# steineggerlab/Metabuli

Hardware: AMD Instinct MI355X
Metric: Mreads/s classified (metabuli classify hot path, reads + index resident in HBM) (higher is better)
Workload: dtype u64

## Files before the change

metabuli_amd/csrc/kernels_score_fast.h:

```cpp
#ifndef MTB_KERNELS_SCORE_FAST_H
#define MTB_KERNELS_SCORE_FAST_H
#include "dev_util.h"
#include "kernels_score.h"
#include "mtb_core.h"
#include "mtb_score_par.h"

#define MTB_FAST_BKT 128
#ifndef MTB_FAST_MERGE_SINGLES
#define MTB_FAST_MERGE_SINGLES 0
#endif

#ifdef MTB_FAST_DEBUG
__device__ unsigned long long mtb_fast_reasons[32];
#define MTB_FAST_COUNT(k, v) do { if (threadIdx.x == 0) atomicAdd(&mtb_fast_reasons[k], (unsigned long long)(v)); } while (0)
#define MTB_FAST_T0() unsigned long long ft_ = __builtin_readcyclecounter()
#define MTB_FAST_MARK(k) do { const unsigned long long t_ = __builtin_readcyclecounter(); if (threadIdx.x == 0) s_ph[k] += t_ - ft_; ft_ = t_; } while (0)
#else
#define MTB_FAST_COUNT(k, v) do {} while (0)
#define MTB_FAST_T0() do {} while (0)
#define MTB_FAST_MARK(k) do {} while (0)
#endif

#define MTB_DPP_RED(v, OP) do { \
    { const uint32_t o_ = (uint32_t)__builtin_amdgcn_update_dpp((int)(v), (int)(v), 0x111, 0xF, 0xF, false); (v) = OP((v), o_); } \
    { const uint32_t o_ = (uint32_t)__builtin_amdgcn_update_dpp((int)(v), (int)(v), 0x112, 0xF, 0xF, false); (v) = OP((v), o_); } \
    { const uint32_t o_ = (uint32_t)__builtin_amdgcn_update_dpp((int)(v), (int)(v), 0x114, 0xF, 0xF, false); (v) = OP((v), o_); } \
    { const uint32_t o_ = (uint32_t)__builtin_amdgcn_update_dpp((int)(v), (int)(v), 0x118, 0xF, 0xF, false); (v) = OP((v), o_); } \
    { const uint32_t o_ = (uint32_t)__builtin_amdgcn_update_dpp((int)(v), (int)(v), 0x142, 0xA, 0xF, false); (v) = OP((v), o_); } \
    { const uint32_t o_ = (uint32_t)__builtin_amdgcn_update_dpp((int)(v), (int)(v), 0x143, 0xC, 0xF, false); (v) = OP((v), o_); } } while (0)
#define MTB_MINU(a, b) ((b) < (a) ? (b) : (a))
#define MTB_MAXU(a, b) ((b) > (a) ? (b) : (a))
__device__ __forceinline__ uint32_t wave_min_u32(uint32_t v) { MTB_DPP_RED(v, MTB_MINU); return (uint32_t)__builtin_amdgcn_readlane((int)v, 63); }
__device__ __forceinline__ uint32_t wave_max_u32(uint32_t v) { MTB_DPP_RED(v, MTB_MAXU); return (uint32_t)__builtin_amdgcn_readlane((int)v, 63); }

struct FKey { uint32_t lo, hi; };
__device__ __forceinline__ uint32_t fk_species(const FKey &k) { return k.hi >> 10; }
__device__ __forceinline__ uint32_t fk_frame(const FKey &k) { return (k.hi >> 7) & 7u; }
__device__ __forceinline__ uint32_t fk_pos(const FKey &k) { return ((k.hi & 127u) << 4) | (k.lo >> 27); }
__device__ __forceinline__ uint32_t fk_ham(const FKey &k) { return (k.lo >> 24) & 7u; }
__device__ __forceinline__ uint32_t fk_dna(const FKey &k) { return k.lo & 0xFFFFFFu; }

struct FastPath { int32_t start, end; float score; int32_t ham; uint32_t rehs;  int32_t species; };

template <int K, int KL = K, bool BYFRAME = false>
__global__ __launch_bounds__(64, K <= 3 ? 5 : 4) void k_score_fast(const mtb_slot16 *__restrict__ slots_all, uint64_t n_reads, const int32_t *__restrict__ qlen,
                                                       const int32_t *__restrict__ qlen2, mtb_tax_view tx, mtb_score_params sp,
                                                       const uint64_t *__restrict__ tc_off, mtb_result *__restrict__ results,
                                                       int32_t *__restrict__ tc_tax, uint32_t *__restrict__ tc_cnt, uint64_t tc_cap, uint64_t tc_base,
                                                       const uint32_t *__restrict__ cursor, uint32_t stride, uint32_t direct, uint32_t epoch,
                                                       uint8_t *__restrict__ slow_flag, uint32_t *__restrict__ cnt_out) {
    constexpr int NMAX = 64 * K;
    __shared__ FKey s_key[NMAX];
    __shared__ uint64_t s_aux[NMAX];
    __shared__ uint64_t s_pp[NMAX];
    __shared__ FastPath s_path[64];
    __shared__ uint32_t s_pf[64];
    __shared__ uint32_t s_tl[(BYFRAME || MTB_FAST_MERGE_SINGLES) ? 64 : 1];
    typedef uint32_t __attribute__((may_alias)) u32a; typedef int32_t __attribute__((may_alias)) i32a;
    static_assert(NMAX * 8 >= 2 * MTB_FAST_BKT * 4 && NMAX * 8 >= 256 * 4 && NMAX * 8 >= (MTB_LR_MAXE + MTB_LR_MAXE * MTB_LR_K) * 4, "tables fit the arrays they live in");
    u32a *const s_hcnt = (u32a *)s_pp;
    u32a *const s_hmin = (u32a *)s_key; i32a *const s_btax = (i32a *)s_key + MTB_FAST_BKT;
    i32a *const s_otax = (i32a *)s_pp; u32a *const s_ocnt = (u32a *)s_pp + MTB_FAST_BKT;
    i32a *const s_lev = (i32a *)s_aux; i32a *const s_anc = (i32a *)s_aux + MTB_LR_MAXE;
    const int32_t lane = (int32_t)threadIdx.x;
    MTB_BEGIN_ACQUIRE();
#ifdef MTB_FAST_DEBUG
    __shared__ unsigned long long s_ph[16];
    if (threadIdx.x < 16) s_ph[threadIdx.x] = 0;
#endif
    const uint64_t lt = lanemask_lt();
    const uint64_t le = lt | (1ull << lane);
    const uint32_t tail_cap = stride - direct;
    const uint32_t div_m = (65536u + (uint32_t)sp.dna_shift - 1u) / (uint32_t)sp.dna_shift;
    const uint32_t lines = (stride * (uint32_t)sizeof(mtb_slot16) + 127u) / 128u;

    for (uint64_t r = blockIdx.x; r < n_reads; r += gridDim.x) {
        if (r + gridDim.x < n_reads && (uint32_t)lane < lines) {
            const uint8_t *pf = (const uint8_t *)(slots_all + (r + gridDim.x) * (uint64_t)stride) + (uint64_t)lane * 128u;
            __builtin_amdgcn_global_load_lds((const __attribute__((address_space(1))) void *)pf, (__attribute__((address_space(3))) void *)s_pf, 4, 0, 0);
        }
        MTB_FAST_T0();
        const int32_t ql1 = qlen[r], ql2 = qlen2[r];
        const int32_t read_len = ql1 + ql2;
        const int32_t nb = mtb_num_buckets(read_len, sp.dna_shift);
        const uint32_t cur = cursor[r];
        const mtb_slot16 *slots = slots_all + r * (uint64_t)stride;
        mtb_slot16 x[KL];
#pragma unroll
        for (int k = 0; k < KL; k++) { const uint32_t i = (uint32_t)lane + 64u * k; x[k].a = 0; x[k].b = 0; if (i < stride) x[k] = slots[i]; }
        bool slow = cur > tail_cap || nb > MTB_FAST_BKT;
        wave_fence();
        MTB_FAST_MARK(0);
        int32_t n = 0, n_live = 0;
        uint32_t spc[KL]; bool live[KL]; int32_t dst[KL];
        uint32_t smin = 0xFFFFFFFFu, smax = 0u;
#pragma unroll
        for (int k = 0; k < KL; k++) {
            const uint32_t i = (uint32_t)lane + 64u * k;
            live[k] = i < stride && mtb_slot_epoch(x[k]) == epoch && (i < direct || i - direct < cur);
            spc[k] = live[k] ? (uint32_t)(x[k].a >> 32) : 0xFFFFFFFFu;
            dst[k] = 0;
            n_live += (int32_t)__popcll(__ballot(live[k]));
            smin = spc[k] < smin ? spc[k] : smin;
            if (live[k]) smax = spc[k] > smax ? spc[k] : smax;
        }
        smin = wave_min_u32(smin); smax = wave_max_u32(smax);
        uint32_t todo_min = 0xFFFFFFFFu;
        if (smin != smax) {
            for (int32_t q = lane; q < 256; q += 64) s_hcnt[q] = 0;
            wave_fence();
#pragma unroll
            for (int k = 0; k < KL; k++) if (live[k]) atomicAdd(&s_hcnt[(spc[k] * 0x9E3779B1u) >> 24], 1u);
            wave_fence();
#pragma unroll
            for (int k = 0; k < KL; k++) if (live[k] && s_hcnt[(spc[k] * 0x9E3779B1u) >> 24] < 2u) { live[k] = false; spc[k] = 0xFFFFFFFFu; }
        } else if (n_live < 2) {
#pragma unroll
            for (int k = 0; k < KL; k++) { live[k] = false; spc[k] = 0xFFFFFFFFu; }
        }
        if (BYFRAME) {
#pragma unroll
            for (int k = 0; k < KL; k++) if (live[k]) spc[k] = (spc[k] << 3) | ((uint32_t)(x[k].b >> 52) & 7u);
        }
#pragma unroll
        for (int k = 0; k < KL; k++) todo_min = spc[k] < todo_min ? spc[k] : todo_min;
        for (int round = 0; ; round++) {
            const uint32_t m = wave_min_u32(todo_min);
            if (m == 0xFFFFFFFFu) break;
            if (round == 24) { slow = true; break; }
            todo_min = 0xFFFFFFFFu;
#pragma unroll
            for (int k = 0; k < KL; k++) {
                const bool mine = spc[k] == m;
                const uint64_t mask = __ballot(mine);
                if (mine) { dst[k] = n + (int32_t)__popcll(mask & lt); spc[k] = 0xFFFFFFFFu; }
                n += (int32_t)__popcll(mask);
                todo_min = spc[k] < todo_min ? spc[k] : todo_min;
            }
        }
        if (KL > K && n > NMAX) slow = true;
#pragma unroll
        for (int k = 0; k < KL; k++) {
            if (live[k] && !slow) {
                const uint64_t b = x[k].b;
                const uint32_t bh = (uint32_t)(b >> 32), ps_ = (bh >> 8) & 0x7FFu;
                FKey fk; fk.hi = ((uint32_t)(x[k].a >> 32) << 10) | (((bh >> 20) & 7u) << 7) | (ps_ >> 4);
                fk.lo = ((ps_ & 15u) << 27) | (((bh >> 23) & 7u) << 24) | ((uint32_t)b & 0xFFFFFFu);
                s_key[dst[k]] = fk;
                s_aux[dst[k]] = (x[k].a & 0xFFFFFFFFull) | (((b >> 24) & 0xFFFFull) << 32) | ((uint32_t)lane + 64u * k >= direct ? (1ull << 63) : 0ull);
            }
        }
        MTB_FAST_MARK(1);
        mtb_result R = mtb_result_blank(ql1, ql2, (uint32_t)tc_base);
        if (!slow && n == 0) { if (lane == 0) { cnt_out[r] = (uint32_t)n_live; results[r] = R; } continue; }
        wave_fence();
        {
            uint32_t nt = 0;
            bool any_tail = false;
#pragma unroll
            for (int k = 0; k < KL; k++) any_tail |= live[k] && (uint32_t)lane + 64u * k >= direct;
            if ((BYFRAME || MTB_FAST_MERGE_SINGLES) && !slow && __any(any_tail)) {
                FKey ke[K]; uint64_t ax[K]; int32_t np[K]; bool tl[K];
                const int32_t nsl = (n + 63) >> 6;
#pragma unroll
                for (int k = 0; k < K; k++) {
                    const int32_t i = lane + 64 * k;
                    ke[k].lo = 0; ke[k].hi = 0; ax[k] = 0; np[k] = i; tl[k] = false;
                    if (k < nsl && i < n) { ke[k] = s_key[i]; ax[k] = s_aux[i]; tl[k] = (ax[k] >> 63) != 0; }
                    if (k < nsl) {
                        const uint64_t tm = __ballot(tl[k]);
                        if (tl[k]) { const uint32_t at = nt + (uint32_t)__popcll(tm & lt); if (at < 64u) s_tl[at] = (uint32_t)i; }
                        nt += (uint32_t)__popcll(tm);
                    }
                }
                if (nt > 64u) slow = true;
                wave_fence();
                if (!slow) {
                    auto same_run = [&](const FKey &a, const FKey &b) { return BYFRAME ? ((a.hi ^ b.hi) >> 7) == 0 : ((a.hi ^ b.hi) >> 10) == 0; };
                    auto less = [&](const FKey &a, const FKey &b) { return a.hi < b.hi || (a.hi == b.hi && a.lo < b.lo); };
                    for (uint32_t t = 0; t < nt; t++) {
                        const int32_t ti = (int32_t)s_tl[t];
                        const FKey kt = s_key[ti];
                        uint32_t n_dir_less = 0, n_dir_run = 0;
#pragma unroll
                        for (int k = 0; k < K; k++) {
                            if (k < nsl) {
                                const int32_t i = lane + 64 * k;
                                const bool dir = i < n && !tl[k] && same_run(ke[k], kt);
                                const bool smaller = dir && less(ke[k], kt);
                                if (dir && !smaller) np[k]++;
                                n_dir_run += (uint32_t)__popcll(__ballot(dir)); n_dir_less += (uint32_t)__popcll(__ballot(smaller));
                            }
                        }
                        uint32_t n_tl_less = 0, n_tl_before = 0;
                        for (uint32_t u = 0; u < nt; u++) {
                            if (u == t) continue;
                            const FKey ku = s_key[s_tl[u]];
                            if (!same_run(ku, kt)) continue;
                            n_tl_less += (less(ku, kt) || (!less(kt, ku) && u < t)) ? 1u : 0u; n_tl_before += u < t ? 1u : 0u;
                        }
                        const int32_t run_start = ti - (int32_t)n_dir_run - (int32_t)n_tl_before;
#pragma unroll
                        for (int k = 0; k < K; k++) if (lane + 64 * k == ti) np[k] = run_start + (int32_t)(n_dir_less + n_tl_less);
                    }
                    wave_fence();
#pragma unroll
                    for (int k = 0; k < K; k++) { const int32_t i = lane + 64 * k; if (k < nsl && i < n) { s_key[np[k]] = ke[k]; s_aux[np[k]] = ax[k] & ~(1ull << 63); } }
                    wave_fence();
                }
            }
        }
        FKey key[K]; uint32_t tid[K], reh[K];
        int32_t tcanon[K]; uint8_t euk[K];
        const mtb_tax_node *nodes = (const mtb_tax_node *)tx.node;
        bool bhead[K], linked[K];
        int32_t shv[K];
        uint64_t bmask[K + 1], lmask[K + 1], rmask[K];
        const int32_t nslot = (n + 63) >> 6;
        bool bad = false, bad2 = false;
#ifdef MTB_FAST_DEBUG
        if (slow) MTB_FAST_COUNT(cur > tail_cap || nb > MTB_FAST_BKT ? 0 : 1, 1);
#endif
#pragma unroll
        for (int k = 0; k < K; k++) {
            const int32_t i = lane + 64 * k;
            key[k].lo = 0; key[k].hi = 0; tid[k] = 0; reh[k] = 0; bhead[k] = true; linked[k] = false; shv[k] = 0; tcanon[k] = -1; euk[k] = 0;
            bmask[k] = ~0ull; lmask[k] = 0; rmask[k] = 0;
            if (k < nslot && !slow) {
                FKey pk; pk.lo = 0; pk.hi = 0;
                if (i < n) {
                    key[k] = s_key[i]; const uint64_t a = s_aux[i]; tid[k] = (uint32_t)a; reh[k] = (uint32_t)(a >> 32) & 0xFFFFu; if (i > 0) pk = s_key[i - 1];
                }
                {
                    const int32_t t_ = (int32_t)tid[k], s_ = (int32_t)fk_species(key[k]);
                    const bool tv = i < n && t_ >= 0 && t_ <= tx.max_taxid, sv = i < n && s_ >= 0 && s_ <= tx.max_taxid;
                    const int32_t tc_ = nodes[tv ? t_ : 0].canon; const uint8_t eu_ = tx.under_euk[sv ? s_ : 0];
                    tcanon[k] = tv ? tc_ : -1; euk[k] = sv ? eu_ : 0;
                }
                const bool first = i == 0;
                if (i < n && !first) {
                    if (pk.hi > key[k].hi || (pk.hi == key[k].hi && pk.lo > key[k].lo)) bad = true;
                    if (pk.hi == key[k].hi && ((pk.lo ^ key[k].lo) >> 27) == 0) bad2 = true;
                }
                bhead[k] = i >= n || first || ((pk.hi ^ key[k].hi) >> 7) != 0;
                if (i < n && !bhead[k]) {
                    const int32_t pos = (int32_t)fk_pos(key[k]), ppos = (int32_t)fk_pos(pk);
                    const int32_t s = (pos - ppos) / 3;
                    if (s > 0 && s <= sp.max_codon_shift) {
                        shv[k] = s;
                        const bool fwd = fk_frame(key[k]) < 3u;
                        linked[k] = mtb_consecutive(fk_dna(pk), fk_dna(key[k]), s, fwd, sp.kmer_format);
                    }
                }
                bmask[k] = __ballot(bhead[k]);
                lmask[k] = __ballot(linked[k]);
                rmask[k] = __ballot(i < n && !linked[k]);
            }
        }
        bmask[K] = ~0ull; lmask[K] = 0;
#ifdef MTB_FAST_DEBUG
        if (!slow) { if (__any(bad)) MTB_FAST_COUNT(2, 1); else if (__any(bad2)) MTB_FAST_COUNT(3, 1); }
#endif
        slow = slow || __any(bad || bad2);
        if (slow) { if (lane == 0) slow_flag[r] = cur > tail_cap ? 2 : 1; continue; }
        if (lane == 0) cnt_out[r] = (uint32_t)n_live;
        MTB_FAST_MARK(2);
        float ps[K]; int32_t phd[K]; int32_t root[K];
        bool cand[K];
        {
            float carry_s = 0.0f; int32_t carry_hd = 0, last_root = 0;
#pragma unroll
            for (int k = 0; k < K; k++) {
                ps[k] = 0.0f; phd[k] = 0; root[k] = 0; cand[k] = false;
                if (k < nslot) {
                    const int32_t i = lane + 64 * k;
                    float is = 0.0f; int32_t ihd = 0;
                    if (linked[k]) mtb_link_inc(reh[k], shv[k], &is, &ihd);
                    ps[k] = wave_inclusive_scan_dpp(is) + carry_s; phd[k] = wave_inclusive_scan_dpp(ihd) + carry_hd;
                    carry_s = rl_f(ps[k], 63); carry_hd = rl_i(phd[k], 63);
                    const uint64_t mr = rmask[k];
                    const uint64_t lo_roots = mr & le;
                    root[k] = lo_roots ? 64 * k + 63 - (int32_t)__builtin_clzll(lo_roots) : last_root;
                    if (mr) last_root = 64 * k + 63 - (int32_t)__builtin_clzll(mr);
                    if (i < n) s_pp[i] = (uint64_t)__float_as_uint(ps[k]) | ((uint64_t)(uint32_t)phd[k] << 32);
                    const uint64_t bnext = (bmask[k] >> 1) | ((bmask[k + 1] & 1ull) << 63);
                    const uint64_t lnext = (lmask[k] >> 1) | ((lmask[k + 1] & 1ull) << 63);
                    const bool has_next = !((bnext >> lane) & 1ull);
                    const bool conn = (lnext >> lane) & 1ull;
                    cand[k] = i < n && (!bhead[k] || has_next) && !conn;
                }
            }
        }
        wave_fence();
        MTB_FAST_MARK(3);
        int32_t ne = 0;
        bool too_many = false;
#pragma unroll
        for (int k = 0; k < K; k++) {
            if (k < nslot) {
                bool e = false;
                FastPath P; P.start = 0; P.end = 0; P.score = 0.0f; P.ham = 0; P.rehs = 0; P.species = 0;
                if (cand[k]) {
                    const int32_t spc = (int32_t)fk_species(key[k]);
                    const int32_t md = euk[k] ? sp.min_cons_cnt_euk : sp.min_cons_cnt;
                    const int32_t rt = root[k];
                    const uint64_t pr = s_pp[rt]; const FKey rkey = s_key[rt];
                    const uint32_t rreh = (uint32_t)(s_aux[rt] >> 32);
                    const int32_t dhd = phd[k] - (int32_t)(uint32_t)(pr >> 32);
                    const int32_t depth = 1 + mtb_link_depth(dhd);
                    if (depth >= md) {
                        e = true;
                        P.start = (int32_t)fk_pos(rkey);
                        P.end = (int32_t)fk_pos(key[k]) + 23;
                        P.score = mtb_part_score(rreh, 8, false) + (rt == lane + 64 * k ? 0.0f : ps[k] - __uint_as_float((uint32_t)pr));
                        P.ham = (int32_t)fk_ham(rkey) + (rt == lane + 64 * k ? 0 : mtb_link_ham(dhd));
                        P.rehs = rreh | (reh[k] << 16);
                        P.species = spc;
                    }
                }
                const uint64_t me = __ballot(e);
                const int32_t at = ne + (int32_t)__popcll(me & lt);
                if (e && at < 64) s_path[at] = P;
                ne += (int32_t)__popcll(me);
            }
        }
        too_many = ne > 64;
        if (too_many) MTB_FAST_COUNT(4, 1); else { MTB_FAST_COUNT(5, 1); MTB_FAST_COUNT(6, ne); }
        if (too_many) { if (lane == 0) slow_flag[r] = 1; continue; }
        if (ne == 0) { if (lane == 0) results[r] = R; continue; }
        wave_fence();
        MTB_FAST_MARK(4);
        FastPath P = s_path[lane < ne ? lane : 0];
        const bool have = lane < ne;
        int32_t prev_spc = __shfl_up(P.species, 1, 64);
        const bool shead = have && (lane == 0 || prev_spc != P.species);
        const uint64_t hmask = __ballot(shead);
        const int32_t nsp = (int32_t)__popcll(hmask);
        MTB_FAST_COUNT(7, nsp);

        float sp_score = -1.0f; int32_t sp_id = 0;
        int32_t s_idx = 0;
        const uint32_t ord = __float_as_uint(P.score);
        const uint32_t tie = ((uint32_t)(1023 - (P.ham < 1023 ? P.ham : 1023)) << 17) | ((uint32_t)(P.start & 0x7FF) << 6) | (uint32_t)(63 - lane);
        for (uint64_t hm = hmask; hm; hm &= hm - 1, s_idx++) {
            const int32_t slo = (int32_t)__builtin_ctzll(hm);
            const int32_t shi = (hm & (hm - 1)) ? (int32_t)__builtin_ctzll(hm & (hm - 1)) : ne;
            const bool in = lane >= slo && lane < shi;
            const uint32_t mh = wave_max_u32(in ? ord : 0u);
            const uint32_t ml = wave_max_u32(in && ord == mh ? tie : 0u);
            const int32_t bl = 63 - (int32_t)(ml & 63u);
            const int32_t f_st = rl_i(P.start, bl), f_en = rl_i(P.end, bl);
            bool surv = in;
            if (in && lane != bl && !((P.end < f_st) || (f_en < P.start))) {
                const int32_t ov = (P.end < f_en ? P.end : f_en) - (P.start > f_st ? P.start : f_st) + 1;
                if (mtb_overlap_drops(ov, P.end - P.start + 1)) surv = false;
            }
            const uint64_t smask = __ballot(surv);
            int32_t rank = 0;
            for (uint64_t fm = smask; fm; fm &= fm - 1) {
                const int32_t f = (int32_t)__builtin_ctzll(fm);
                const float fs = rl_f(P.score, f); const int32_t fh = rl_i(P.ham, f), fst = rl_i(P.start, f);
                const bool before = fs != P.score ? fs > P.score : (fh != P.ham ? fh < P.ham : (fst != P.start ? fst > P.start : f < lane));
                rank += (f != lane && before) ? 1 : 0;
            }
            const int32_t ns = (int32_t)__popcll(smask);
            int32_t acc_st = 0, acc_en = 0, na = 0; float sum = 0.0f;
            for (int32_t q = 0; q < ns; q++) {
                const int32_t o = (int32_t)__builtin_ctzll(__ballot(surv && rank == q));
                struct { int32_t start, end; float score; int32_t ham; } c;
                c.start = rl_i(P.start, o); c.end = rl_i(P.end, o); c.ham = rl_i(P.ham, o); c.score = rl_f(P.score, o);
                const uint32_t crehs = (uint32_t)rl_i((int32_t)P.rehs, o);
                bool drop = false;
                uint64_t ovm = __ballot(lane < na && !((c.end < acc_st) || (acc_en < c.start)));
                while (ovm && !drop) {
                    const int32_t a2 = (int32_t)__builtin_ctzll(ovm); ovm &= ovm - 1;
                    drop = mtb_path_against(c, rl_i(acc_st, a2), rl_i(acc_en, a2), [&] { return crehs >> 16; }, [&] { return crehs & 0xFFFFu; });
                }
                if (!drop) { if (lane == na) { acc_st = c.start; acc_en = c.end; } na++; sum += c.score; }
            }
            float sc = sum / (float)read_len; sc = sc < 1.0f ? sc : 1.0f;
            const int32_t spid = rl_i(P.species, slo);
            if (lane == s_idx) { sp_score = sc; sp_id = spid; }
        }
        MTB_FAST_MARK(5);
        const bool valid = lane < nsp && !(sp_score < sp.min_score);
        const int32_t meaningful = (int32_t)__popcll(__ballot(valid && sp_score > 0.0f));
        if (meaningful == 0) { if (lane == 0) results[r] = R; continue; }
        float best_sp = valid ? sp_score : -1.0f;
#pragma unroll
        for (int d = 32; d > 0; d >>= 1) { const float o2 = __shfl_xor(best_sp, d, 64); best_sp = o2 > best_sp ? o2 : best_sp; }
        const float cut = best_sp * sp.tie_ratio;
        mtb_tie tie_sp = mtb_tie_none();
        for (uint64_t tm = __ballot(valid && sp_score >= cut); tm; tm &= tm - 1) {
            const int32_t s = (int32_t)__builtin_ctzll(tm);
            mtb_tie_add(&tx, &tie_sp, rl_i(sp_id, s), rl_f(sp_score, s));
        }
        if (!mtb_tie_decide(&tie_sp, &sp, &R)) { if (lane == 0) results[r] = R; continue; }
        const int32_t species = tie_sp.only;
        const bool sp_ok = species >= 0 && species <= tx.max_taxid;
        mtb_tax_node rs = nodes[sp_ok ? species : 0];
        if (!sp_ok) { rs.canon = -1; rs.depth = 0; rs.parent = -1; rs.flags = 0; }
        MTB_FAST_MARK(6);
        for (int32_t q = lane; q < nb; q += 64) { s_hmin[q] = 255u; s_btax[q] = -1; }
        wave_fence();
        int32_t bq[K];
#pragma unroll
        for (int k = 0; k < K; k++) {
            bq[k] = -1;
            if (k < nslot) {
                const int32_t i = lane + 64 * k;
                if (i < n && (int32_t)fk_species(key[k]) == species) {
                    const int32_t q = (int32_t)((fk_pos(key[k]) * div_m) >> 16);
                    if (q < nb) { bq[k] = q; atomicMin(&s_hmin[q], fk_ham(key[k])); }
                }
            }
        }
        wave_fence();
#pragma unroll
        for (int k = 0; k < K; k++) {
            if (k < nslot && bq[k] >= 0 && fk_ham(key[k]) == s_hmin[bq[k]]) {
                const int32_t t = (int32_t)tid[k];
                const int32_t tc = tcanon[k] < 0 ? t : tcanon[k];
                mtb_bucket_merge(&s_btax[bq[k]], t, [&tx, tc](int32_t a, int32_t b) { return a == b ? tc : mtb_lca(&tx, a, b); });
            }
        }
        wave_fence();
        const uint64_t off = tc_off[r], room = tc_off[r + 1] - off;
        MTB_FAST_MARK(7);
        int32_t ntc = 0;
        {
            uint32_t t0 = 0xFFFFFFFFu, t1 = 0xFFFFFFFFu;
            if (lane < nb && s_hmin[lane] != 255u) t0 = (uint32_t)s_btax[lane];
            if (lane + 64 < nb && s_hmin[lane + 64] != 255u) t1 = (uint32_t)s_btax[lane + 64];
            while (ntc < (int32_t)room) {
                const uint32_t mn = wave_min_u32(t0 < t1 ? t0 : t1);
                if (mn == 0xFFFFFFFFu) break;
                const uint32_t cnt = (uint32_t)__popcll(__ballot(t0 == mn)) + (uint32_t)__popcll(__ballot(t1 == mn));
                if (lane == 0) { s_otax[ntc] = (int32_t)mn; s_ocnt[ntc] = cnt; }
                if (t0 == mn) t0 = 0xFFFFFFFFu;
                if (t1 == mn) t1 = 0xFFFFFFFFu;
                ntc++;
            }
        }
        wave_fence();
        MTB_FAST_MARK(8);
        int32_t slow_lr = ntc > MTB_LR_MAXE ? 1 : 0;
        if (!slow_lr && lane < ntc) {
            const int32_t tax = s_otax[lane];
            const bool t_ok = tax >= 0 && tax <= tx.max_taxid;
            mtb_tax_node rt = nodes[t_ok ? tax : 0];
            if (!t_ok) { rt.canon = -1; rt.depth = 0; rt.parent = -1; rt.flags = 0; }
            int32_t lv;
            const int32_t cs = rs.canon, c = rt.canon;
            if (cs < 0 || c < 0) lv = -1;
            else {
                const int32_t L = rt.depth - rs.depth;
                if (L < 0) lv = -1;
                else if (L > MTB_LR_K) lv = MTB_LR_K + 1;
                else {
                    int32_t a = c;
                    for (int32_t k = L - 1; k >= 0; k--) { s_anc[lane * MTB_LR_K + k] = a; a = (k == L - 1) ? rt.parent : tx.parent[a]; }
                    lv = (a == cs) ? L : -1;
                }
            }
            s_lev[lane] = lv;
            if (lv > MTB_LR_K) slow_lr = 1;
        }
        slow_lr = __any(slow_lr) ? 1 : 0;
        wave_fence();
        if (lane == 0) {
            R.n_taxcnt = (uint16_t)ntc;
            R.classification = mtb_finish_taxon(&tx, &sp, species, rs.canon, R.score, slow_lr != 0, s_lev, s_anc, s_otax, s_ocnt, ntc, read_len);
            R.taxcnt_off = (uint32_t)(off + tc_base);
            for (int32_t k = 0; k < ntc; k++)
                if (off + k < tc_cap) { tc_tax[off + k] = s_otax[k]; tc_cnt[off + k] = s_ocnt[k]; }
            results[r] = R;
        }
        MTB_FAST_MARK(9);
    }
#ifdef MTB_FAST_DEBUG
    __syncthreads();
    if (threadIdx.x < 16) atomicAdd(&mtb_fast_reasons[8 + threadIdx.x], s_ph[threadIdx.x]);
#endif
}

#endif
```

metabuli_amd/csrc/kernels_score_many.h:

```cpp
#ifndef MTB_KERNELS_SCORE_MANY_H
#define MTB_KERNELS_SCORE_MANY_H
#include "dev_util.h"
#include "mtb_core.h"
#include "kernels_join.h"
#include "kernels_score.h"
#include "kernels_score_long.h"
#include "kernels_seg_order.h"

#define MTB_MANY_CLAIM 16u
#define MTB_MANY_HASH 1024u

__global__ __launch_bounds__(256) void k_ovf_count(const uint32_t *__restrict__ cursor, const uint8_t *__restrict__ off, uint64_t n_reads, uint32_t tail_cap,
                                                    uint32_t *__restrict__ novf) {
    const uint64_t r = (uint64_t)blockIdx.x * 256 + threadIdx.x;
    if (r >= n_reads) return;
    const uint32_t cur = cursor[r];
    const uint32_t n = (cur > tail_cap && !(off && off[r])) ? cur - tail_cap : 0u;
    novf[r] = n <= 65535u ? n : 0u;
}
__global__ __launch_bounds__(256) void k_ovf_group(const mtb_match *__restrict__ ovf, uint64_t n_ovf, const uint64_t *__restrict__ start, const uint32_t *__restrict__ novf,
                                                    uint32_t *__restrict__ ocur, mtb_match *__restrict__ out, uint64_t region_cap, const unsigned long long *__restrict__ counters) {
    uint64_t i = (uint64_t)blockIdx.x * 256 + threadIdx.x;
    if (region_cap) {
        const unsigned long long cnt = counters[8 * blockIdx.y];
        if (i >= cnt || i >= region_cap) return;
        i += (uint64_t)blockIdx.y * region_cap;
    } else if (i >= n_ovf) return;
    mtb_match m = ovf[i];
    const uint32_t r = mtb_q_seq(m.qinfo) - 1;
    const uint32_t cap = novf[r];
    if (!cap) return;
    uint32_t at;
    if (m.pad & 2u) { at = (uint32_t)(m.qinfo >> 16) & 0xFFFFu; m.qinfo &= ~0xFFFF0000ull; m.pad = 0; }
    else at = atomicAdd(&ocur[r], 1u);
    if (at < cap) out[start[r] + at] = m;
}

#define MTB_MSORT_NT 256
template <int LOG2HASH, uint32_t MAXN>
__global__ __launch_bounds__(MTB_MSORT_NT) void k_many_sort(const mtb_slot16 *__restrict__ slots_all, uint32_t stride, uint32_t direct, uint32_t epoch,
                                                             const uint32_t *__restrict__ cursor, const uint8_t *__restrict__ off_reads,
                                                             const mtb_match *__restrict__ ovfg, const uint64_t *__restrict__ ovf_start,
                                                             const uint32_t *__restrict__ list, uint32_t n_list, const int32_t *__restrict__ qlen, const int32_t *__restrict__ qlen2,
                                                             int32_t dna_shift, const uint64_t *__restrict__ big_start, mtb_match *__restrict__ big, uint32_t *__restrict__ seg_cnt,
                                                             uint8_t *__restrict__ todo, uint32_t only_flag, uint32_t beyond_flag ) {
    constexpr uint32_t HASH = 1u << LOG2HASH;
    __shared__ __attribute__((aligned(16))) uint64_t s_u[HASH];
    __shared__ uint16_t s_idx[MAXN];
    __shared__ uint32_t s_n, s_full;
    static_assert(MAXN * 8 <= HASH * 8, "the sort keys live in the table's storage");
    uint32_t *const h_key = (uint32_t *)s_u, *const h_val = h_key + HASH;
    const uint32_t tid = threadIdx.x, lane = tid & 63u;
    const uint64_t lt = lanemask_lt();
    const uint32_t tail_cap = stride - direct;
    for (uint32_t b = blockIdx.x; b < n_list; b += gridDim.x) {
        const uint64_t r = (uint64_t)list[b];
        if (only_flag && todo[r] != only_flag) continue;
        const uint32_t cur = cursor[r], tail_n = cur < tail_cap ? cur : tail_cap;
        uint64_t o0 = 0; uint32_t n_ov = 0;
        if (ovf_start) { o0 = ovf_start[r]; n_ov = (uint32_t)(ovf_start[r + 1] - o0); }
        const int32_t nb = mtb_num_buckets(qlen[r] + qlen2[r], dna_shift);
        const bool skip = (off_reads && off_reads[r]) || cur - tail_n != n_ov || stride + n_ov > 65535u || nb > 256;
        __syncthreads();
        if (only_flag && tid == 0) todo[r] = 0;
        if (skip) { if (tid == 0) { seg_cnt[b] = 0; todo[r] = 1; } continue; }
        for (uint32_t q = tid; q < HASH; q += MTB_MSORT_NT) { h_key[q] = 0xFFFFFFFFu; h_val[q] = 0u; }
        if (tid == 0) { s_n = 0; s_full = 0; }
        __syncthreads();
        const mtb_slot16 *slots = slots_all + r * (uint64_t)stride;
        const uint32_t n_src = stride + n_ov;
        auto probe = [&](uint32_t i, uint32_t *sp_, uint32_t *fr_) -> bool {
            if (i < stride) { const mtb_slot16 x = slots[i]; *sp_ = (uint32_t)(x.a >> 32); *fr_ = (uint32_t)(x.b >> 52) & 7u; return seg_slot_live(x, i, direct, tail_n, epoch); }
            const mtb_match m = ovfg[o0 + (i - stride)]; *sp_ = (uint32_t)m.species_id; *fr_ = mtb_q_frame(m.qinfo); return true;
        };
        for (uint32_t i = tid; i < n_src; i += MTB_MSORT_NT) {
            uint32_t s_, f_;
            if (!probe(i, &s_, &f_)) continue;
            if (*(volatile uint32_t *)&s_full) break;
            uint32_t h = (s_ * 0x9E3779B1u) >> (32 - LOG2HASH); bool done = false;
            for (uint32_t p = 0; p < HASH && !done; p++) {
                const uint32_t old = atomicCAS(&h_key[h], 0xFFFFFFFFu, s_);
                if (old == 0xFFFFFFFFu || old == s_) { const uint32_t bit = 1u << f_; if (atomicOr(&h_val[h], bit) & bit) atomicOr(&h_val[h], bit << 8); done = true; }
                h = (h + 1u) & (HASH - 1u);
            }
            if (!done) s_full = 1;
        }
        __syncthreads();
        uint32_t used = 0;
        for (uint32_t q = tid; q < HASH; q += MTB_MSORT_NT) used += h_key[q] != 0xFFFFFFFFu ? 1u : 0u;
        if (used) atomicAdd(&s_n, used);
        __syncthreads();
        const bool over = s_full || s_n > HASH / 4u * 3u;
        __syncthreads();
        if (over) { if (tid == 0) { seg_cnt[b] = 0; todo[r] = (uint8_t)beyond_flag; } continue; }
        if (tid == 0) s_n = 0;
        __syncthreads();
        for (uint32_t i0 = 0; i0 < n_src; i0 += MTB_MSORT_NT) {
            const uint32_t i = i0 + tid;
            bool keep = false;
            if (i < n_src) {
                uint32_t s_, f_;
                if (probe(i, &s_, &f_)) {
                    uint32_t h = (s_ * 0x9E3779B1u) >> (32 - LOG2HASH);
                    for (uint32_t p = 0; p < HASH; p++) { const uint32_t k = h_key[h]; if (k == s_) { keep = (h_val[h] >> 8) != 0u; break; } if (k == 0xFFFFFFFFu) break; h = (h + 1u) & (HASH - 1u); }
                }
            }
            const uint64_t km = __ballot(keep);
            if (km) {
                uint32_t at0 = 0;
                if (lane == 0) at0 = atomicAdd(&s_n, (uint32_t)__popcll(km));
                at0 = (uint32_t)__shfl((int)at0, 0, 64);
                if (keep) { const uint32_t at = at0 + (uint32_t)__popcll(km & lt); if (at < MAXN) s_idx[at] = (uint16_t)i; }
            }
        }
        __syncthreads();
        const uint32_t n = s_n;
        __syncthreads();
        if (n > MAXN) { if (tid == 0) { seg_cnt[b] = 0; todo[r] = (uint8_t)beyond_flag; } continue; }
        auto fetch = [&](uint32_t i) -> mtb_match {
            if (i < stride) return mtb_slot_unpack(slots[i], (uint32_t)r + 1);
            mtb_match m = ovfg[o0 + (i - stride)]; m.pad = 0; return m;
        };
        for (uint32_t j = tid; j < n; j += MTB_MSORT_NT) {
            const mtb_match m = fetch(s_idx[j]);
            s_u[j] = ((uint64_t)(uint32_t)m.species_id << 41) | ((uint64_t)mtb_q_frame(m.qinfo) << 38) | ((uint64_t)(mtb_q_pos(m.qinfo) & 0x7FFu) << 27) |
                     ((uint64_t)(m.hamming & 7u) << 24) | (m.dna & 0xFFFFFFu);
        }
        __syncthreads();
        so_bitonic(s_u, s_idx, n, tid);
        mtb_match *dst = big + big_start[b];
        for (uint32_t j = tid; j < n; j += MTB_MSORT_NT) {
            const mtb_match m = fetch(s_idx[j]);
            uint64_t *d = (uint64_t *)(dst + j); const uint64_t *q = (const uint64_t *)&m;
            d[0] = q[0]; d[1] = q[1]; d[2] = q[2];
        }
        if (tid == 0) seg_cnt[b] = n;
    }
}
__global__ __launch_bounds__(256) void k_list_flagged(const uint32_t *__restrict__ list, uint32_t n_list, const uint8_t *__restrict__ todo, const uint32_t *__restrict__ big_cnt,
                                                       uint32_t *__restrict__ rest, uint32_t *__restrict__ n_rest, uint32_t *__restrict__ cnt_out) {
    const uint32_t b = blockIdx.x * 256 + threadIdx.x;
    if (b >= n_list) return;
    const uint32_t r = list[b];
    if (todo[r]) rest[atomicAdd(n_rest, 1u)] = r;
    else cnt_out[r] = big_cnt[b];
}

template <bool KEY64, int CAP>
__global__ __launch_bounds__(64, (CAP > 192 ? 2 : 3)) void k_score_many(const mtb_slot16 *__restrict__ slots_all, uint32_t stride, uint32_t direct, uint32_t epoch,
                                                       const uint32_t *__restrict__ cursor, const uint8_t *__restrict__ off_reads,
                                                       const mtb_match *__restrict__ ovfg, const uint64_t *__restrict__ ovf_start,
                                                       const uint32_t *__restrict__ list, const uint32_t *__restrict__ n_list,
                                                       const int32_t *__restrict__ qlen, const int32_t *__restrict__ qlen2, mtb_tax_view tx, mtb_score_params sp,
                                                       const uint64_t *__restrict__ tc_off, mtb_result *__restrict__ results, int32_t *__restrict__ tc_tax,
                                                       uint32_t *__restrict__ tc_cnt, uint64_t tc_cap, uint64_t tc_base,
                                                       uint32_t *__restrict__ rest_list, uint32_t *__restrict__ n_rest, uint32_t *__restrict__ cnt_out,
                                                       unsigned long long *__restrict__ work, unsigned long long *__restrict__ stats ) {
    __shared__ __attribute__((aligned(16))) uint8_t s_ws[MTB_SCORE_WS_BYTES_(CAP)];
    static_assert(MTB_SCORE_WS_BYTES_(CAP) - CAP * sizeof(mtb_match) >= MTB_MANY_HASH * 8, "the species table fits behind the match records");
    static_assert(CAP * sizeof(mtb_path) >= MTB_SCORE_BKT * 13 + (MTB_LR_MAXE + MTB_LR_MAXE * MTB_LR_K) * 4, "decide arrays must fit the path area");
    uint32_t *const h_key = (uint32_t *)(s_ws + CAP * sizeof(mtb_match));
    uint32_t *const h_val = h_key + MTB_MANY_HASH;
    __shared__ uint32_t s_tfull;
    const uint32_t lane = threadIdx.x;
    const uint64_t lt = lanemask_lt();
    const uint32_t tail_cap = stride - direct;
    MTB_BEGIN_ACQUIRE();
    const uint64_t n_iter = (uint64_t)*n_list;
    unsigned long long seen = 0, kept = 0;
    for (uint64_t c0 = (uint64_t)__shfl(lane == 0 ? atomicAdd(work, (unsigned long long)MTB_MANY_CLAIM) : 0ull, 0, 64); c0 < n_iter;
         c0 = (uint64_t)__shfl(lane == 0 ? atomicAdd(work, (unsigned long long)MTB_MANY_CLAIM) : 0ull, 0, 64))
    for (uint64_t it = c0; it < c0 + MTB_MANY_CLAIM && it < n_iter; it++) {
        const uint64_t r = (uint64_t)list[it];
        const int32_t ql1 = qlen[r], ql2 = qlen2[r];
        const int32_t read_len = ql1 + ql2;
        const int32_t nb = mtb_num_buckets(read_len, sp.dna_shift);
        const uint32_t cur = cursor[r];
        const uint32_t tail_n = cur < tail_cap ? cur : tail_cap;
        uint64_t o0 = 0; uint32_t n_ov = 0;
        if (ovf_start) { o0 = ovf_start[r]; n_ov = (uint32_t)(ovf_start[r + 1] - o0); }
        bool hand_on = (off_reads && off_reads[r]) || nb > MTB_SCORE_BKT || cur - tail_n != n_ov;
        uint32_t why = 2;
        if (!hand_on && cur > 3u * (uint32_t)CAP) { hand_on = true; why = 4; }
        const mtb_slot16 *slots = slots_all + r * (uint64_t)stride;
        mtb_sws<uint16_t> w;
        mtb_sws_carve<uint16_t>(&w, s_ws, CAP);
        uint32_t n = 0, n_all = 0;
        if (!hand_on) {
            score_sync<uint16_t>();
            for (uint32_t q = lane; q < MTB_MANY_HASH; q += 64) { h_key[q] = 0xFFFFFFFFu; h_val[q] = 0u; }
            if (lane == 0) s_tfull = 0;
            score_sync<uint16_t>();
            bool full = false;
            auto enter = [&](uint32_t s, uint32_t f) {
                if (*(volatile uint32_t *)&s_tfull) { full = true; return; }
                uint32_t h = (s * 0x9E3779B1u) >> 22;
                for (uint32_t p = 0; p < MTB_MANY_HASH; p++) {
                    const uint32_t old = atomicCAS(&h_key[h], 0xFFFFFFFFu, s);
                    if (old == 0xFFFFFFFFu || old == s) {
                        const uint32_t bit = 1u << f;
                        if (atomicOr(&h_val[h], bit) & bit) atomicOr(&h_val[h], bit << 8);
                        return;
                    }
                    h = (h + 1u) & (MTB_MANY_HASH - 1u);
                }
                full = true; s_tfull = 1;
            };
            for (uint32_t c0 = 0; c0 < stride; c0 += 64) {
                const uint32_t i = c0 + lane;
                mtb_slot16 x; x.a = 0; x.b = 0;
                if (i < stride) x = slots[i];
                const bool live = i < stride && seg_slot_live(x, i, direct, tail_n, epoch);
                if (live) enter((uint32_t)(x.a >> 32), (uint32_t)(x.b >> 52) & 7u);
                n_all += (uint32_t)__popcll(__ballot(live));
            }
            for (uint32_t c0 = 0; c0 < n_ov; c0 += 64) {
                const uint32_t i = c0 + lane;
                if (i < n_ov) { const mtb_match m = ovfg[o0 + i]; enter((uint32_t)m.species_id, mtb_q_frame(m.qinfo)); }
            }
            n_all += n_ov;
            score_sync<uint16_t>();
            uint32_t used = 0;
            for (uint32_t q = lane; q < MTB_MANY_HASH; q += 64) used += h_key[q] != 0xFFFFFFFFu ? 1u : 0u;
            for (int d = 32; d > 0; d >>= 1) used += (uint32_t)__shfl_xor((int)used, d, 64);
            hand_on = __any(full) || used > MTB_MANY_HASH / 4u * 3u;
            why = 3;
            if (!hand_on) {
                auto alive = [&](uint32_t s) -> bool {
                    uint32_t h = (s * 0x9E3779B1u) >> 22;
                    for (uint32_t p = 0; p < MTB_MANY_HASH; p++) {
                        const uint32_t k = h_key[h];
                        if (k == s) return (h_val[h] >> 8) != 0u;
                        if (k == 0xFFFFFFFFu) return false;
                        h = (h + 1u) & (MTB_MANY_HASH - 1u);
                    }
                    return false;
                };
                uint64_t *dst64 = (uint64_t *)w.m;
                auto put = [&](uint32_t pos, const mtb_match &m) {
                    const uint64_t *q = (const uint64_t *)&m;
                    dst64[3 * pos] = q[0]; dst64[3 * pos + 1] = q[1]; dst64[3 * pos + 2] = q[2];
                };
                for (uint32_t c0 = 0; c0 < stride; c0 += 64) {
                    const uint32_t i = c0 + lane;
                    mtb_slot16 x; x.a = 0; x.b = 0;
                    if (i < stride) x = slots[i];
                    const bool keep = i < stride && seg_slot_live(x, i, direct, tail_n, epoch) && alive((uint32_t)(x.a >> 32));
                    const uint64_t mask = __ballot(keep);
                    const uint32_t pos = n + (uint32_t)__popcll(mask & lt);
                    if (keep && pos < (uint32_t)CAP) put(pos, mtb_slot_unpack(x, (uint32_t)r + 1));
                    n += (uint32_t)__popcll(mask);
                }
                for (uint32_t c0 = 0; c0 < n_ov; c0 += 64) {
                    const uint32_t i = c0 + lane;
                    mtb_match m; m.qinfo = 0; m.target_id = 0; m.species_id = 0; m.dna = 0; m.right_end_hamming = 0; m.hamming = 0; m.pad = 0;
                    bool keep = false;
                    if (i < n_ov) { m = ovfg[o0 + i]; keep = alive((uint32_t)m.species_id); }
                    const uint64_t mask = __ballot(keep);
                    const uint32_t pos = n + (uint32_t)__popcll(mask & lt);
                    if (keep && pos < (uint32_t)CAP) { m.pad = 0; put(pos, m); }
                    n += (uint32_t)__popcll(mask);
                }
                hand_on = n > (uint32_t)CAP;
                why = 4;
                score_sync<uint16_t>();
            }
        }
        if (hand_on) { if (lane == 0) { rest_list[atomicAdd(n_rest, 1u)] = (uint32_t)r; if (stats) atomicAdd(&stats[why], 1ull); } continue; }
        seen += n_all; kept += n;
        mtb_result R = mtb_result_blank(ql1, ql2, 0);
        if (lane == 0) cnt_out[r] = n_all;
        if (n == 0) { if (lane == 0) results[r] = R; continue; }
        const uint64_t off = tc_off[r], room = tc_off[r + 1] - off;
        int32_t *s_btax = (int32_t *)w.path, *s_otax = s_btax + MTB_SCORE_BKT;
        uint32_t *s_ocnt = (uint32_t *)(s_otax + MTB_SCORE_BKT);
        int32_t *s_lev = (int32_t *)(s_ocnt + MTB_SCORE_BKT), *s_anc = s_lev + MTB_LR_MAXE;
        uint8_t *s_bham = (uint8_t *)(s_anc + MTB_LR_MAXE * MTB_LR_K);
        score_read_par<uint16_t, true, KEY64, mtb_match, true, CAP>(w.m, (int32_t)n, w, s_btax, s_bham, s_otax, s_ocnt, s_lev, s_anc, nb, read_len, tx, sp, off, room,
                                                                   tc_tax, tc_cnt, tc_cap, (mtb_match *)nullptr, R);
        if (lane == 0) { R.query_length = ql1; R.query_length2 = ql2; R.reserved = 0; R.taxcnt_off += (uint32_t)tc_base; results[r] = R; }
    }
    if (stats && lane == 0 && seen) { atomicAdd(&stats[0], seen); atomicAdd(&stats[1], kept); }
}

#endif
```

Baseline: 70.80.

## Enable singles merge with parallel rank placement and batch per-read metadata loads

```diff
diff --git a/metabuli_amd/csrc/kernels_score_fast.h b/metabuli_amd/csrc/kernels_score_fast.h
--- a/metabuli_amd/csrc/kernels_score_fast.h
+++ b/metabuli_amd/csrc/kernels_score_fast.h
@@ -7,7 +7,7 @@
 
 #define MTB_FAST_BKT 128
 #ifndef MTB_FAST_MERGE_SINGLES
-#define MTB_FAST_MERGE_SINGLES 0
+#define MTB_FAST_MERGE_SINGLES 1
 #endif
 
 #ifdef MTB_FAST_DEBUG
@@ -162,50 +162,58 @@
             if ((BYFRAME || MTB_FAST_MERGE_SINGLES) && !slow && __any(any_tail)) {
                 FKey ke[K]; uint64_t ax[K]; int32_t np[K]; bool tl[K];
                 const int32_t nsl = (n + 63) >> 6;
+                auto same_run = [&](const FKey &a, const FKey &b) { return BYFRAME ? ((a.hi ^ b.hi) >> 7) == 0 : ((a.hi ^ b.hi) >> 10) == 0; };
+                auto less = [&](const FKey &a, const FKey &b) { return a.hi < b.hi || (a.hi == b.hi && a.lo < b.lo); };
+                bool unsorted = false;
 #pragma unroll
                 for (int k = 0; k < K; k++) {
                     const int32_t i = lane + 64 * k;
                     ke[k].lo = 0; ke[k].hi = 0; ax[k] = 0; np[k] = i; tl[k] = false;
-                    if (k < nsl && i < n) { ke[k] = s_key[i]; ax[k] = s_aux[i]; tl[k] = (ax[k] >> 63) != 0; }
+                    if (k < nsl && i < n) {
+                        ke[k] = s_key[i]; ax[k] = s_aux[i]; tl[k] = (ax[k] >> 63) != 0;
+                        if (i > 0 && !tl[k]) { const FKey pk = s_key[i - 1]; if ((s_aux[i - 1] >> 63) == 0 && same_run(pk, ke[k]) && less(ke[k], pk)) unsorted = true; }
+                    }
                     if (k < nsl) {
                         const uint64_t tm = __ballot(tl[k]);
                         if (tl[k]) { const uint32_t at = nt + (uint32_t)__popcll(tm & lt); if (at < 64u) s_tl[at] = (uint32_t)i; }
                         nt += (uint32_t)__popcll(tm);
                     }
                 }
-                if (nt > 64u) slow = true;
+                if (nt > 64u || __any(unsorted)) slow = true;
                 wave_fence();
                 if (!slow) {
-                    auto same_run = [&](const FKey &a, const FKey &b) { return BYFRAME ? ((a.hi ^ b.hi) >> 7) == 0 : ((a.hi ^ b.hi) >> 10) == 0; };
-                    auto less = [&](const FKey &a, const FKey &b) { return a.hi < b.hi || (a.hi == b.hi && a.lo < b.lo); };
-                    for (uint32_t t = 0; t < nt; t++) {
-                        const int32_t ti = (int32_t)s_tl[t];
-                        const FKey kt = s_key[ti];
-                        uint32_t n_dir_less = 0, n_dir_run = 0;
-#pragma unroll
-                        for (int k = 0; k < K; k++) {
-                            if (k < nsl) {
-                                const int32_t i = lane + 64 * k;
-                                const bool dir = i < n && !tl[k] && same_run(ke[k], kt);
-                                const bool smaller = dir && less(ke[k], kt);
-                                if (dir && !smaller) np[k]++;
-                                n_dir_run += (uint32_t)__popcll(__ballot(dir)); n_dir_less += (uint32_t)__popcll(__ballot(smaller));
-                            }
-                        }
-                        uint32_t n_tl_less = 0, n_tl_before = 0;
-                        for (uint32_t u = 0; u < nt; u++) {
-                            if (u == t) continue;
-                            const FKey ku = s_key[s_tl[u]];
-                            if (!same_run(ku, kt)) continue;
-                            n_tl_less += (less(ku, kt) || (!less(kt, ku) && u < t)) ? 1u : 0u; n_tl_before += u < t ? 1u : 0u;
-                        }
-                        const int32_t run_start = ti - (int32_t)n_dir_run - (int32_t)n_tl_before;
-#pragma unroll
-                        for (int k = 0; k < K; k++) if (lane + 64 * k == ti) np[k] = run_start + (int32_t)(n_dir_less + n_tl_less);
-                    }
+                    const bool mine = (uint32_t)lane < nt;
+                    const int32_t ti = mine ? (int32_t)s_tl[lane] : 0;
+                    const FKey kt = s_key[ti]; const uint64_t at = s_aux[ti];
+                    uint32_t n_tl_run = 0, n_tl_less = 0;
+                    for (uint32_t u = 0; u < nt; u++) {
+                        FKey ku; ku.hi = (uint32_t)rl_i((int32_t)kt.hi, (int32_t)u); ku.lo = (uint32_t)rl_i((int32_t)kt.lo, (int32_t)u);
+                        if (same_run(ku, kt)) { n_tl_run++; n_tl_less += (less(ku, kt) || (!less(kt, ku) && u < (uint32_t)lane)) ? 1u : 0u; }
+#pragma unroll
+                        for (int k = 0; k < K; k++)
+                            if (k < nsl && !tl[k] && same_run(ke[k], ku) && !less(ke[k], ku)) np[k]++;
+                    }
+                    const uint32_t rid = BYFRAME ? kt.hi >> 7 : kt.hi >> 10;
+                    int32_t lo0 = 0, hi0 = n, lo1 = 0, hi1 = n;
+                    for (int32_t len = n; len; len >>= 1) {
+                        const int32_t m0 = (lo0 + hi0) >> 1, m1 = (lo1 + hi1) >> 1;
+                        const uint32_t r0 = BYFRAME ? s_key[m0 < n ? m0 : 0].hi >> 7 : s_key[m0 < n ? m0 : 0].hi >> 10;
+                        const uint32_t r1 = BYFRAME ? s_key[m1 < n ? m1 : 0].hi >> 7 : s_key[m1 < n ? m1 : 0].hi >> 10;
+                        if (lo0 < hi0) { if (r0 < rid) lo0 = m0 + 1; else hi0 = m0; }
+                        if (lo1 < hi1) { if (r1 <= rid) lo1 = m1 + 1; else hi1 = m1; }
+                    }
+                    const int32_t run_start = lo0, n_dir_run = lo1 - lo0 - (int32_t)n_tl_run;
+                    int32_t lo2 = run_start, hi2 = run_start + n_dir_run;
+                    for (int32_t len = n; len; len >>= 1) {
+                        const int32_t m2 = (lo2 + hi2) >> 1;
+                        const FKey km = s_key[m2 < n ? m2 : 0];
+                        if (lo2 < hi2) { if (less(km, kt)) lo2 = m2 + 1; else hi2 = m2; }
+                    }
+                    const int32_t place = lo2 + (int32_t)n_tl_less;
                     wave_fence();
 #pragma unroll
-                    for (int k = 0; k < K; k++) { const int32_t i = lane + 64 * k; if (k < nsl && i < n) { s_key[np[k]] = ke[k]; s_aux[np[k]] = ax[k] & ~(1ull << 63); } }
+                    for (int k = 0; k < K; k++) { const int32_t i = lane + 64 * k; if (k < nsl && i < n && !tl[k]) { s_key[np[k]] = ke[k]; s_aux[np[k]] = ax[k]; } }
+                    if (mine) { s_key[place] = kt; s_aux[place] = at & ~(1ull << 63); }
                     wave_fence();
                 }
             }
diff --git a/metabuli_amd/csrc/kernels_score_many.h b/metabuli_amd/csrc/kernels_score_many.h
--- a/metabuli_amd/csrc/kernels_score_many.h
+++ b/metabuli_amd/csrc/kernels_score_many.h
@@ -169,26 +169,58 @@
     const uint64_t n_iter = (uint64_t)*n_list;
     unsigned long long seen = 0, kept = 0;
     for (uint64_t c0 = (uint64_t)__shfl(lane == 0 ? atomicAdd(work, (unsigned long long)MTB_MANY_CLAIM) : 0ull, 0, 64); c0 < n_iter;
-         c0 = (uint64_t)__shfl(lane == 0 ? atomicAdd(work, (unsigned long long)MTB_MANY_CLAIM) : 0ull, 0, 64))
-    for (uint64_t it = c0; it < c0 + MTB_MANY_CLAIM && it < n_iter; it++) {
-        const uint64_t r = (uint64_t)list[it];
-        const int32_t ql1 = qlen[r], ql2 = qlen2[r];
+         c0 = (uint64_t)__shfl(lane == 0 ? atomicAdd(work, (unsigned long long)MTB_MANY_CLAIM) : 0ull, 0, 64)) {
+    const uint32_t n_blk = (uint32_t)(n_iter - c0 < (uint64_t)MTB_MANY_CLAIM ? n_iter - c0 : (uint64_t)MTB_MANY_CLAIM);
+    uint32_t h_r = 0, h_cur = 0, h_nov = 0, h_ql = 0; uint64_t h_o0 = 0;
+    if (lane < n_blk) {
+        h_r = list[c0 + lane];
+        const uint32_t q1 = (uint32_t)qlen[h_r], q2 = (uint32_t)qlen2[h_r];
+        h_ql = (q1 < 65535u ? q1 : 65535u) | ((q2 < 65535u ? q2 : 65535u) << 16); h_cur = cursor[h_r];
+        uint64_t o1 = 0; uint8_t routed = 0;
+        if (ovf_start) { h_o0 = ovf_start[h_r]; o1 = ovf_start[(uint64_t)h_r + 1]; }
+        if (off_reads) routed = off_reads[h_r];
+        h_nov = routed ? 0xFFFFFFFFu : (uint32_t)(o1 - h_o0);
+    }
+    auto rl_u64 = [](uint64_t v, int32_t l) { return (uint64_t)(uint32_t)rl_i((int32_t)(uint32_t)v, l) | ((uint64_t)(uint32_t)rl_i((int32_t)(uint32_t)(v >> 32), l) << 32); };
+    for (uint32_t j = 0; j < n_blk; j++) {
+        const uint64_t r = (uint64_t)(uint32_t)rl_i((int32_t)h_r, (int32_t)j);
+        const uint32_t qlp = (uint32_t)rl_i((int32_t)h_ql, (int32_t)j);
+        const int32_t ql1 = (int32_t)(qlp & 0xFFFFu), ql2 = (int32_t)(qlp >> 16);
         const int32_t read_len = ql1 + ql2;
         const int32_t nb = mtb_num_buckets(read_len, sp.dna_shift);
-        const uint32_t cur = cursor[r];
+        const uint32_t cur = (uint32_t)rl_i((int32_t)h_cur, (int32_t)j);
         const uint32_t tail_n = cur < tail_cap ? cur : tail_cap;
-        uint64_t o0 = 0; uint32_t n_ov = 0;
-        if (ovf_start) { o0 = ovf_start[r]; n_ov = (uint32_t)(ovf_start[r + 1] - o0); }
-        bool hand_on = (off_reads && off_reads[r]) || nb > MTB_SCORE_BKT || cur - tail_n != n_ov;
+        const uint64_t o0 = rl_u64(h_o0, (int32_t)j);
+        const uint32_t n_ov = (uint32_t)rl_i((int32_t)h_nov, (int32_t)j);
+        bool hand_on = n_ov == 0xFFFFFFFFu || nb > MTB_SCORE_BKT || cur - tail_n != n_ov;
         uint32_t why = 2;
         if (!hand_on && cur > 3u * (uint32_t)CAP) { hand_on = true; why = 4; }
         const mtb_slot16 *slots = slots_all + r * (uint64_t)stride;
         mtb_sws<uint16_t> w;
         mtb_sws_carve<uint16_t>(&w, s_ws, CAP);
         uint32_t n = 0, n_all = 0;
+        constexpr bool REGS = CAP <= 192;
+        const bool in_regs = REGS && stride <= 192u;
+        uint64_t xa[REGS ? 3 : 1], xb[REGS ? 3 : 1], ow[REGS ? 2 : 1][3];
+        auto ow_species = [](const uint64_t *w_) { return (uint32_t)(w_[1] >> 32); };
+        static_assert(sizeof(mtb_match) == 24 && offsetof(mtb_match, species_id) == 12 && offsetof(mtb_match, pad) == 23, "overflow entries are read as three 64-bit words");
         if (!hand_on) {
+            if constexpr (REGS) if (in_regs) {
+#pragma unroll
+                for (int k = 0; k < 3; k++) { const uint32_t i = lane + 64u * k; xa[k] = 0; xb[k] = 0; if (i < stride) { const mtb_slot16 x = slots[i]; xa[k] = x.a; xb[k] = x.b; } }
+#pragma unroll
+                for (int k = 0; k < 2; k++) {
+                    const uint32_t i = lane + 64u * k;
+                    ow[k][0] = 0; ow[k][1] = 0; ow[k][2] = 0;
+                    if (i < n_ov) { const uint64_t *q = (const uint64_t *)(ovfg + o0 + i); ow[k][0] = q[0]; ow[k][1] = q[1]; ow[k][2] = q[2]; }
+                }
+            }
             score_sync<uint16_t>();
-            for (uint32_t q = lane; q < MTB_MANY_HASH; q += 64) { h_key[q] = 0xFFFFFFFFu; h_val[q] = 0u; }
+            {
+                uint4 *const tb = (uint4 *)h_key;
+                const uint4 ones = make_uint4(0xFFFFFFFFu, 0xFFFFFFFFu, 0xFFFFFFFFu, 0xFFFFFFFFu), zero = make_uint4(0u, 0u, 0u, 0u);
+                for (uint32_t q = lane; q < MTB_MANY_HASH / 4u; q += 64) { tb[q] = ones; tb[q + MTB_MANY_HASH / 4u] = zero; }
+            }
             if (lane == 0) s_tfull = 0;
             score_sync<uint16_t>();
             bool full = false;
@@ -206,6 +238,19 @@
                 }
                 full = true; s_tfull = 1;
             };
+            if constexpr (REGS) if (in_regs) {
+#pragma unroll
+                for (int k = 0; k < 3; k++) {
+                    const uint32_t i = lane + 64u * k;
+                    mtb_slot16 x; x.a = xa[k]; x.b = xb[k];
+                    const bool live = i < stride && seg_slot_live(x, i, direct, tail_n, epoch);
+                    if (live) enter((uint32_t)(x.a >> 32), (uint32_t)(x.b >> 52) & 7u);
+                    n_all += (uint32_t)__popcll(__ballot(live));
+                }
+#pragma unroll
+                for (int k = 0; k < 2; k++) if (lane + 64u * k < n_ov) enter(ow_species(ow[k]), mtb_q_frame(ow[k][0]));
+            }
+            if (!in_regs)
             for (uint32_t c0 = 0; c0 < stride; c0 += 64) {
                 const uint32_t i = c0 + lane;
                 mtb_slot16 x; x.a = 0; x.b = 0;
@@ -214,7 +259,7 @@
                 if (live) enter((uint32_t)(x.a >> 32), (uint32_t)(x.b >> 52) & 7u);
                 n_all += (uint32_t)__popcll(__ballot(live));
             }
-            for (uint32_t c0 = 0; c0 < n_ov; c0 += 64) {
+            for (uint32_t c0 = in_regs ? 128u : 0u; c0 < n_ov; c0 += 64) {
                 const uint32_t i = c0 + lane;
                 if (i < n_ov) { const mtb_match m = ovfg[o0 + i]; enter((uint32_t)m.species_id, mtb_q_frame(m.qinfo)); }
             }
@@ -241,6 +286,29 @@
                     const uint64_t *q = (const uint64_t *)&m;
                     dst64[3 * pos] = q[0]; dst64[3 * pos + 1] = q[1]; dst64[3 * pos + 2] = q[2];
                 };
+                if constexpr (REGS) if (in_regs) {
+#pragma unroll
+                    for (int k = 0; k < 3; k++) {
+                        const uint32_t i = lane + 64u * k;
+                        mtb_slot16 x; x.a = xa[k]; x.b = xb[k];
+                        const bool keep = i < stride && seg_slot_live(x, i, direct, tail_n, epoch) && alive((uint32_t)(x.a >> 32));
+                        const uint64_t mask = __ballot(keep);
+                        const uint32_t pos = n + (uint32_t)__popcll(mask & lt);
+                        if (keep && pos < (uint32_t)CAP) put(pos, mtb_slot_unpack(x, (uint32_t)r + 1));
+                        n += (uint32_t)__popcll(mask);
+                    }
+#pragma unroll
+                    for (int k = 0; k < 2; k++) {
+                        if (64u * k < n_ov) {
+                            const bool keep = lane + 64u * k < n_ov && alive(ow_species(ow[k]));
+                            const uint64_t mask = __ballot(keep);
+                            const uint32_t pos = n + (uint32_t)__popcll(mask & lt);
+                            if (keep && pos < (uint32_t)CAP) { dst64[3 * pos] = ow[k][0]; dst64[3 * pos + 1] = ow[k][1]; dst64[3 * pos + 2] = ow[k][2] & ~(0xFFull << 56); }
+                            n += (uint32_t)__popcll(mask);
+                        }
+                    }
+                }
+                if (!in_regs)
                 for (uint32_t c0 = 0; c0 < stride; c0 += 64) {
                     const uint32_t i = c0 + lane;
                     mtb_slot16 x; x.a = 0; x.b = 0;
@@ -251,7 +319,7 @@
                     if (keep && pos < (uint32_t)CAP) put(pos, mtb_slot_unpack(x, (uint32_t)r + 1));
                     n += (uint32_t)__popcll(mask);
                 }
-                for (uint32_t c0 = 0; c0 < n_ov; c0 += 64) {
+                for (uint32_t c0 = in_regs ? 128u : 0u; c0 < n_ov; c0 += 64) {
                     const uint32_t i = c0 + lane;
                     mtb_match m; m.qinfo = 0; m.target_id = 0; m.species_id = 0; m.dna = 0; m.right_end_hamming = 0; m.hamming = 0; m.pad = 0;
                     bool keep = false;
@@ -280,6 +348,7 @@
                                                                    tc_tax, tc_cnt, tc_cap, (mtb_match *)nullptr, R);
         if (lane == 0) { R.query_length = ql1; R.query_length2 = ql2; R.reserved = 0; R.taxcnt_off += (uint32_t)tc_base; results[r] = R; }
     }
+    }
     if (stats && lane == 0 && seen) { atomicAdd(&stats[0], seen); atomicAdd(&stats[1], kept); }
 }
 
```

Measured after the change: 72.59 (median of 6 runs). 2.5% higher.
